# daooshee/ReReVST-Code

Measured on AMD Instinct MI355X. Metric: stylized frames/sec at 512x512, 1 style, higher is better.
Workload: dtype f32

## Files before the change

### rerevst-code_amd/csrc/conv_f43.h

```cpp
#pragma once
#include "conv_wino.h"

#ifndef F43_ABL
#define F43_ABL 0
#endif
#ifndef F43_SPAN
#define F43_SPAN 28
#endif

typedef float f32x2 __attribute__((ext_vector_type(2)));

struct F43Geo {
    static constexpr int NT = 256;
    static constexpr int NPOS = 36;
    static constexpr int RAW_ROW_BYTES = 4 * 9 * 32;
    static constexpr int RAW_PIECES = 34 * 4 * 9 * 2;
    static constexpr int RAW_IT = (RAW_PIECES + NT - 1) / NT;
    static constexpr int RAW_BYTES = RAW_IT * NT * 16;
    static constexpr int U_BYTES = NPOS * 32 * 8 * 4;
    static constexpr int U_IT = U_BYTES / 16 / NT;
    static constexpr int SMEM = 2 * RAW_BYTES + 2 * U_BYTES + WINO_PAR_BYTES;
};

__device__ __forceinline__ f32x2 p2sub(const f32x2 a, const f32x2 b) {
    f32x2 r;
    asm("v_pk_add_f32 %0, %1, %2 neg_lo:[0,1] neg_hi:[0,1]" : "=v"(r) : "v"(a), "v"(b));
    return r;
}
template <int IMM>
__device__ __forceinline__ f32x2 lds_rd64(unsigned addr) {
    static_assert(IMM >= 0 && IMM < 65536, "ds_read offset is a 16-bit unsigned immediate");
    f32x2 r;
    asm volatile("ds_read_b64 %0, %1 offset:%2" : "=v"(r) : "v"(addr), "i"(IMM));
    return r;
}

template <bool AG>
__device__ __forceinline__ void mfma_acc(f32x4& acc, const float a, const float b) {
    if constexpr (AG) asm volatile("v_mfma_f32_16x16x4_f32 %0, %1, %2, %0" : "+a"(acc) : "v"(a), "v"(b));
    else asm volatile("v_mfma_f32_16x16x4_f32 %0, %1, %2, %0" : "+v"(acc) : "v"(a), "v"(b));
}
template <bool AG>
__device__ __forceinline__ void mfma_zero(f32x4& acc, const float a, const float b) {
    if constexpr (AG) asm volatile("v_mfma_f32_16x16x4_f32 %0, %1, %2, 0" : "=a"(acc) : "v"(a), "v"(b));
    else asm volatile("v_mfma_f32_16x16x4_f32 %0, %1, %2, 0" : "=v"(acc) : "v"(a), "v"(b));
}

constexpr float F43_A = 0.75f, F43_B = 1.5f;
constexpr float F43_A2 = F43_A * F43_A, F43_B2 = F43_B * F43_B, F43_P = F43_A2 * F43_B2, F43_S = F43_A2 + F43_B2;
constexpr float F43_A3 = F43_A2 * F43_A, F43_B3 = F43_B2 * F43_B;
constexpr unsigned f43_bits(float f) { return __builtin_bit_cast(unsigned, f); }

struct F43Tmp { f32x2 a, b, c, f, g; };
struct F43K { unsigned long long b2, a2, p, s, a, b; };
__device__ __forceinline__ F43K f43_load_k() {
    F43K k;
    asm volatile("s_mov_b64 %0, %6\n\ts_mov_b64 %1, %7\n\ts_mov_b64 %2, %8\n\ts_mov_b64 %3, %9\n\ts_mov_b64 %4, %10\n\ts_mov_b64 %5, %11"
                 : "=s"(k.b2), "=s"(k.a2), "=s"(k.p), "=s"(k.s), "=s"(k.a), "=s"(k.b)
                 : "i"(f43_bits(F43_B2)), "i"(f43_bits(F43_A2)), "i"(f43_bits(F43_P)), "i"(f43_bits(F43_S)), "i"(f43_bits(F43_A)), "i"(f43_bits(F43_B)));
    return k;
}
template <bool NEG>
__device__ __forceinline__ void fmak3s(f32x2& r0, f32x2& r1, f32x2& r2, const f32x2 x0, const f32x2 x1, const f32x2 x2,
                                       const f32x2 c0, const f32x2 c1, const f32x2 c2, const unsigned long long ks) {
    if constexpr (NEG)
        asm volatile("v_pk_fma_f32 %0, %4, %3, %7 op_sel_hi:[1,0,1] neg_lo:[0,1,0] neg_hi:[0,1,0]\n\tv_pk_fma_f32 %1, %5, %3, %8 op_sel_hi:[1,0,1] neg_lo:[0,1,0] neg_hi:[0,1,0]\n\t"
                     "v_pk_fma_f32 %2, %6, %3, %9 op_sel_hi:[1,0,1] neg_lo:[0,1,0] neg_hi:[0,1,0]"
                     : "=&v"(r0), "=&v"(r1), "=&v"(r2) : "s"(ks), "v"(x0), "v"(x1), "v"(x2), "v"(c0), "v"(c1), "v"(c2));
    else
        asm volatile("v_pk_fma_f32 %0, %4, %3, %7 op_sel_hi:[1,0,1]\n\tv_pk_fma_f32 %1, %5, %3, %8 op_sel_hi:[1,0,1]\n\tv_pk_fma_f32 %2, %6, %3, %9 op_sel_hi:[1,0,1]"
                     : "=&v"(r0), "=&v"(r1), "=&v"(r2) : "s"(ks), "v"(x0), "v"(x1), "v"(x2), "v"(c0), "v"(c1), "v"(c2));
}
template <int LB, class LineFn>
__device__ __forceinline__ void f43_in3s(LineFn&& L, const F43K& k) {
    F43Tmp t[3];
    using N0 = std::integral_constant<int, LB>; using N1 = std::integral_constant<int, LB + 1>; using N2 = std::integral_constant<int, LB + 2>;
    using I0 = std::integral_constant<int, 0>; using I1 = std::integral_constant<int, 1>; using I2 = std::integral_constant<int, 2>;
    using I3 = std::integral_constant<int, 3>; using I4 = std::integral_constant<int, 4>; using I5 = std::integral_constant<int, 5>;
#define F43_D(J) L(N0{}, I##J{}), L(N1{}, I##J{}), L(N2{}, I##J{})
#define F43_T(M) t[0].M, t[1].M, t[2].M
    fmak3s<true>(F43_T(a), F43_D(2), F43_D(4), k.b2);
    fmak3s<true>(F43_T(b), F43_D(1), F43_D(3), k.b2);
    fmak3s<true>(F43_T(c), F43_D(2), F43_D(4), k.a2);
    fmak3s<true>(F43_T(f), F43_D(1), F43_D(3), k.a2);
    fmak3s<false>(F43_T(g), F43_D(0), F43_D(4), k.p);
    fmak3s<true>(F43_D(0), F43_D(2), F43_T(g), k.s);
    fmak3s<false>(F43_T(g), F43_D(1), F43_D(5), k.p);
    fmak3s<true>(F43_D(5), F43_D(3), F43_T(g), k.s);
    fmak3s<false>(F43_D(1), F43_T(b), F43_T(a), k.a);
    fmak3s<true>(F43_D(2), F43_T(b), F43_T(a), k.a);
    fmak3s<false>(F43_D(3), F43_T(f), F43_T(c), k.b);
    fmak3s<true>(F43_D(4), F43_T(f), F43_T(c), k.b);
#undef F43_D
#undef F43_T
}
__device__ __forceinline__ void f43_out(const f32x2 m0, const f32x2 m1, const f32x2 m2, const f32x2 m3, const f32x2 m4, const f32x2 m5,
                                        f32x2& y0, f32x2& y1, f32x2& y2, f32x2& y3) {
    f32x2 s1, d1, s2, d2;
    unsigned long long ks;
    asm volatile(
        "v_pk_add_f32 %[s1], %[m1], %[m2]\n\t"
        "v_pk_add_f32 %[d1], %[m1], %[m2] neg_lo:[0,1] neg_hi:[0,1]\n\t"
        "v_pk_add_f32 %[s2], %[m3], %[m4]\n\t"
        "v_pk_add_f32 %[d2], %[m3], %[m4] neg_lo:[0,1] neg_hi:[0,1]\n\t"
        "v_pk_add_f32 %[y0], %[m0], %[s1]\n\t"
        "s_mov_b64 %[k], %[ka]\n\t"
        "v_pk_mul_f32 %[y1], %[d1], %[k] op_sel_hi:[1,0]\n\t"
        "s_mov_b64 %[k], %[ka2]\n\t"
        "v_pk_mul_f32 %[y2], %[s1], %[k] op_sel_hi:[1,0]\n\t"
        "s_mov_b64 %[k], %[ka3]\n\t"
        "v_pk_fma_f32 %[y3], %[d1], %[k], %[m5] op_sel_hi:[1,0,1]\n\t"
        "v_pk_add_f32 %[y0], %[y0], %[s2]\n\t"
        "s_mov_b64 %[k], %[kb]\n\t"
        "v_pk_fma_f32 %[y1], %[d2], %[k], %[y1] op_sel_hi:[1,0,1]\n\t"
        "s_mov_b64 %[k], %[kb2]\n\t"
        "v_pk_fma_f32 %[y2], %[s2], %[k], %[y2] op_sel_hi:[1,0,1]\n\t"
        "s_mov_b64 %[k], %[kb3]\n\t"
        "v_pk_fma_f32 %[y3], %[d2], %[k], %[y3] op_sel_hi:[1,0,1]"
        : [y0] "=&v"(y0), [y1] "=&v"(y1), [y2] "=&v"(y2), [y3] "=&v"(y3), [s1] "=&v"(s1), [d1] "=&v"(d1), [s2] "=&v"(s2), [d2] "=&v"(d2), [k] "=&s"(ks)
        : [m0] "v"(m0), [m1] "v"(m1), [m2] "v"(m2), [m3] "v"(m3), [m4] "v"(m4), [m5] "v"(m5),
          [ka] "i"(f43_bits(F43_A)), [ka2] "i"(f43_bits(F43_A2)), [ka3] "i"(f43_bits(F43_A3)),
          [kb] "i"(f43_bits(F43_B)), [kb2] "i"(f43_bits(F43_B2)), [kb3] "i"(f43_bits(F43_B3)));
}

#ifndef P8_PAD
#define P8_PAD 6
#define P8_COL0 4
#endif
template <int EPI, int LAY = 0>
__global__ __launch_bounds__(256, 1) void conv_f43_k(const ConvP) {
    static_assert(!(EPI & E_RES), "same-resolution residuals are not needed by the layers this kernel serves");
    constexpr bool INP8 = (LAY & 1) != 0, OUTP8 = (LAY & 2) != 0;
    const ConvPK p0 = conv_args();
    auto wp_of = [](const ConvPK k) { return k->Wi + 2 + (INP8 ? P8_PAD : 0); };
    const int WP = wp_of(p0);
    using G = F43Geo;
    constexpr int ABL = F43_ABL;
    constexpr int RAW_BYTES = G::RAW_BYTES, U_BYTES = G::U_BYTES, NT = G::NT, NPOS = G::NPOS;
    extern __shared__ __attribute__((aligned(16))) char smem[];
    const int tid = threadIdx.x;
    const int wave = __builtin_amdgcn_readfirstlane(tid >> 6);
    const int lane = tid & 63, t = lane & 15, q = lane >> 4;
    const int tr = t >> 3, tc = t & 7;
    const int nchunks = p0->Cin >> 3;

    struct Item { int tx, ty, b, nt; };
    Item cur, nxt, dlt;
    {
        const ConvPK p = p0;
        const int n_ntiles = p->Cout >> 5;
        const int GD = gridDim.x, w = blockIdx.x;
        int pix, dpix;
        if (p->xcd_slabs) {
            const int PT = (GD >> 3) / n_ntiles;
            pix = (w & 7) * PT + (w >> 3) / n_ntiles; dpix = 8 * PT;
            cur.nt = (w >> 3) % n_ntiles; dlt.nt = 0;
        } else {
            cur.nt = w % n_ntiles; pix = w / n_ntiles;
            dlt.nt = GD % n_ntiles; dpix = GD / n_ntiles;
        }
        cur.tx = pix % p->tiles_x; cur.ty = (pix / p->tiles_x) % p->tiles_y; cur.b = pix / (p->tiles_x * p->tiles_y);
        dlt.tx = dpix % p->tiles_x; dlt.ty = (dpix / p->tiles_x) % p->tiles_y; dlt.b = dpix / (p->tiles_x * p->tiles_y);
    }
    auto advance = [&](const ConvPK p, const Item& a) {
        const int n_ntiles = p->Cout >> 5;
        Item r = a;
        r.nt += dlt.nt;
        int carry = 0;
        if (r.nt >= n_ntiles) { r.nt -= n_ntiles; carry = 1; }
        r.tx += dlt.tx + carry;
        if (r.tx >= p->tiles_x) { r.tx -= p->tiles_x; r.ty += 1; }
        r.ty += dlt.ty;
        if (r.ty >= p->tiles_y) { r.ty -= p->tiles_y; r.b += 1; }
        r.b += dlt.b;
        return r;
    };
    auto in_of = [&](const ConvPK p, const Item& a) {
        const int WP = wp_of(p);
        const size_t img_floats = (size_t)(p->Hi + 2) * WP * p->Cin;
        return p->in + (size_t)a.b * img_floats + (size_t)(((a.ty + p->ty0) * 32) * WP + (a.tx + p->tx0) * 32 + (INP8 ? P8_COL0 - 1 : 0)) * (INP8 ? 8 : p->Cin);
    };
    const size_t plane_floats = (size_t)(p0->Hi + 2) * WP * 8;
    auto lim_of = [&](const ConvPK p, const Item& a) {
        const int WP = wp_of(p);
        const long rows_left = (long)(p->Hi + 2) - (long)(a.ty + p->ty0) * 32;
        const long n = (rows_left * WP - (long)(a.tx + p->tx0) * 32 - (INP8 ? P8_COL0 - 1 : 0)) * (INP8 ? 8 : p->Cin) * 4;
        return (int)(n > 0x7fffffffL ? 0x7fffffffL : n);
    };
    auto w_of = [&](const ConvPK p, const Item& a) { return p->wpk + (size_t)a.nt * nchunks * (U_BYTES / 4); };
    int asrc[G::RAW_IT];
#pragma unroll
    for (int it = 0; it < G::RAW_IT; ++it) {
        int e = it * NT + tid;
        if (e >= G::RAW_PIECES) e = 0;
        const int half = e & 1, xd = (e >> 1) % 9, ph = ((e >> 1) / 9) & 3, y = (e >> 1) / 36;
        const int x = 4 * xd + ph, par = (y >> 2) & 1;
        asrc[it] = ((y * WP + x) * (INP8 ? 8 : p0->Cin) + 4 * (half ^ par)) * 4;
        if (ABL & 64) asrc[it] = (it * NT + tid) * 16;
    }
    bool have = cur.b < p0->B, have_nxt = false;
    const float* in_t = in_of(p0, cur);
    const float* w_t = w_of(p0, cur);
    int lim_t = lim_of(p0, cur);
    const float* in_n = in_t;
    const float* w_n = w_t;
    int lim_n = lim_t;
    auto stage_u = [&](int chunk) {
        char* udst = smem + 2 * RAW_BYTES + (chunk & 1) * U_BYTES;
#pragma unroll
        for (int it = 0; it < G::U_IT; ++it) bufld16(w_t, udst + (it * NT + wave * 64) * 16, tid * 16, chunk * U_BYTES + it * NT * 16);
    };
    auto stage_raw = [&](int chunk) {
        char* rdst = smem + (chunk & 1) * RAW_BYTES;
        const rsrc_t rs = make_rsrc(INP8 ? in_t + chunk * plane_floats : in_t, lim_t);
#pragma unroll
        for (int it = 0; it < G::RAW_IT; ++it) bufld16_rs(rs, rdst + (it * NT + wave * 64) * 16, asrc[it], INP8 ? 0 : chunk * 32);
    };
    char* const par = smem + 2 * RAW_BYTES + 2 * U_BYTES;
    auto stage_params = [&](int ntile, int img) {
        if (wave < 2) {
            const ConvPK p = conv_args();
            const int e = tid;
            const int row = e >> 3, col = (e & 7) * 4;
            const float* src = p->bias;
            int off = ntile * 32 + col;
            const int pb = img * p->par_bstride;
            if (row >= 1 && row <= 4) { src = (EPI & E_NORM1) ? p->n1 : p->bias; off += (EPI & E_NORM1) ? (row - 1) * p->Cout + pb : 0; }
            if (row >= 5 && row <= 8) { src = (EPI & E_NORM2) ? p->n2 : p->bias; off += (EPI & E_NORM2) ? (row - 5) * p->Cout + pb : 0; }
            if (row >= 9) { src = (EPI & E_NORM2) ? p->sty : p->bias; off += (EPI & E_NORM2) ? (row - 9) * p->Cout + pb : 0; }
            if (row > 10) { src = p->bias; off = ntile * 32; }
            glds16(src + off, par + wave * 1024);
        }
    };

    const unsigned lds0 = (unsigned)(size_t)(__attribute__((address_space(3))) char*)smem;
    const int y0 = 8 * wave + 4 * tr;
    const unsigned rawA = lds0 + y0 * G::RAW_ROW_BYTES + tc * 32 + ((q ^ (2 * (tr & 1))) << 3);
    const unsigned rawB = lds0 + y0 * G::RAW_ROW_BYTES + tc * 32 + ((q ^ (2 * ((tr & 1) ^ 1))) << 3);
    const unsigned offU = lds0 + 2 * RAW_BYTES + t * 64 + ((q ^ ((0 - (t >> 2)) & 3)) << 4);

#ifndef F43_NAG
#define F43_NAG 28
#endif
    constexpr int NAG = F43_NAG;
    f32x4 accA[NAG][2], accV[NPOS - NAG][2];
    int par_ntile = -1, par_img = -1;
    long long tl[10] = {0, 0, 0, 0, 0, 0, 0, 0, 0, 0}, tl_t = 0, pair_t = 0;
    const long long run_ck = (ABL & 16) ? clock64() : 0, run_rt = (ABL & 16) ? wall_clock64() : 0;
    auto tick = [&](int k) { if (ABL & 16) { const long long n = clock64(); tl[k] += n - tl_t; tl_t = n; } };
    f32x2 v[NPOS];
    f32x4 ur[2][6];
    auto full_transform = [&](f32x2 (&d)[NPOS]) {
        const F43K k = f43_load_k();
        auto col = [&](auto nc, auto jc) -> f32x2& { return d[decltype(nc)::value * 6 + decltype(jc)::value]; };
        auto row = [&](auto nc, auto jc) -> f32x2& { return d[decltype(jc)::value * 6 + decltype(nc)::value]; };
        f43_in3s<0>(col, k);
        f43_in3s<3>(col, k);
        f43_in3s<0>(row, k);
        f43_in3s<3>(row, k);
    };
    auto read_patch_col = [&](auto rbc, auto dxc) {
        constexpr int RB = decltype(rbc)::value, dx = decltype(dxc)::value;
        static_for([&](auto dyc) {
            constexpr int dy = decltype(dyc)::value;
            constexpr int off = RB + dy * G::RAW_ROW_BYTES + (dx & 3) * 288 + (dx >> 2) * 32;
            v[dx * 6 + dy] = lds_rd64<off>(dy < 4 ? rawA : rawB);
        }, std::make_integer_sequence<int, 6>{});
    };
    auto read_u_batch = [&](unsigned ub, auto bc, auto slotc) {
        constexpr int b = decltype(bc)::value, sl = decltype(slotc)::value;
        static_for([&](auto rc) {
            constexpr int r = decltype(rc)::value;
            ur[sl][r] = lds_rd128<(r * 6 + b) * 1024>(ub);
        }, std::make_integer_sequence<int, 6>{});
    };

    auto chunk_body = [&](int c, auto par_c, auto first_c, auto tail_c) {
        constexpr int PAR = decltype(par_c)::value;
        constexpr bool FIRST = decltype(first_c)::value;
        constexpr int TAIL = decltype(tail_c)::value;
        constexpr bool last = TAIL == 2;
        constexpr bool own_u = TAIL < 2, own_r = TAIL < 1;
        const rsrc_t rs_u = make_rsrc(own_u ? w_t : w_n);
        const int rchunk = own_r ? c + 2 : TAIL - 1;
        const rsrc_t rs_r = make_rsrc(INP8 ? (own_r ? in_t : in_n) + rchunk * plane_floats : (own_r ? in_t : in_n), own_r ? lim_t : lim_n);
        const int usoff = own_u ? (c + 1) * U_BYTES : 0;
        const int rsoff = INP8 ? 0 : rchunk * 32;
        int wb = wave * 1024;
        asm volatile("" : "+s"(wb));
        lds_char* const wdst = (lds_char*)smem + wb;
        lds_char* const udst = wdst + 2 * RAW_BYTES + (1 - PAR) * U_BYTES;
        lds_char* const rdst = wdst + PAR * RAW_BYTES;
        const unsigned ub = offU + PAR * U_BYTES;
        const unsigned ubn = offU + (1 - PAR) * U_BYTES;
        using RBt = std::integral_constant<int, (1 - PAR) * RAW_BYTES>;
        static_for([&](auto bc) {
            constexpr int b = decltype(bc)::value;
            if constexpr (b <= 1) asm volatile("s_waitcnt lgkmcnt(0)" ::: "memory");
            else if (last) asm volatile("s_waitcnt lgkmcnt(0)" ::: "memory");
            else asm volatile("s_waitcnt lgkmcnt(6)" ::: "memory");
            if constexpr (b < 5) read_u_batch(ub, std::integral_constant<int, b + 1>{}, std::integral_constant<int, (b + 1) & 1>{});
            static_for([&](auto rc) {
                constexpr int r = decltype(rc)::value, pos = r * 6 + b;
                constexpr int step = b * 6 + r;
                auto dma_req = [&](auto nc) {
                    constexpr int n = decltype(nc)::value;
                    if constexpr (n < G::RAW_IT) bufld16_rs(rs_r, rdst + n * NT * 16, asrc[n], rsoff);
                    else if constexpr (n < G::RAW_IT + G::U_IT) bufld16_rs(rs_u, udst + (n - G::RAW_IT) * NT * 16, tid * 16, usoff + (n - G::RAW_IT) * NT * 16);
                };
                {
                    constexpr int SPAN = F43_SPAN, NREQ = G::RAW_IT + G::U_IT;
                    constexpr int n = (step * NREQ + SPAN - 1) / SPAN;
                    if constexpr (n < NREQ && (n * SPAN) / NREQ == step) { if (!(ABL & 1)) dma_req(std::integral_constant<int, n>{}); }
                }
                if constexpr (r == 3) {
                    if constexpr (b >= 1) { if (!last) read_patch_col(RBt{}, std::integral_constant<int, b - 1>{}); }
                }
                constexpr bool AG = pos < NAG;
                f32x4 (&ac)[2] = *[&]() -> f32x4 (*)[2] { if constexpr (AG) return &accA[pos]; else return &accV[pos - NAG]; }();
                const f32x2 vv = v[b * 6 + r];
                const f32x4 uu = ur[b & 1][r];
                if constexpr (FIRST) { mfma_zero<AG>(ac[0], vv[0], uu[0]); mfma_zero<AG>(ac[1], vv[0], uu[2]); }
                else { mfma_acc<AG>(ac[0], vv[0], uu[0]); mfma_acc<AG>(ac[1], vv[0], uu[2]); }
                mfma_acc<AG>(ac[0], vv[1], uu[1]);
                mfma_acc<AG>(ac[1], vv[1], uu[3]);
            }, std::make_integer_sequence<int, 6>{});
        }, std::make_integer_sequence<int, 6>{});
        if (!last) read_patch_col(RBt{}, std::integral_constant<int, 5>{});
        tick(1);
        if (!(ABL & 2)) asm volatile("s_waitcnt vmcnt(0) lgkmcnt(0)\n\ts_barrier" ::: "memory");
        else asm volatile("s_waitcnt lgkmcnt(0)" ::: "memory");
        tick(3);
        if (!last) {
            read_u_batch(ubn, std::integral_constant<int, 0>{}, std::integral_constant<int, 0>{});
            if (!(ABL & 8)) full_transform(v);
        }
        tick(5);
    };

    auto next_patch = [&]() {
        static_for([&](auto dxc) { read_patch_col(std::integral_constant<int, 0>{}, dxc); }, std::make_integer_sequence<int, 6>{});
        read_u_batch(offU, std::integral_constant<int, 0>{}, std::integral_constant<int, 0>{});
        if (!(ABL & 2)) asm volatile("s_waitcnt lgkmcnt(0)\n\ts_barrier" ::: "memory");
        else asm volatile("s_waitcnt lgkmcnt(0)" ::: "memory");
        if (!(ABL & 8)) full_transform(v);
    };
    if (have) {
        stage_raw(0);
        stage_u(0);
        stage_raw(1);
        stage_params(cur.nt, cur.b);
        par_ntile = cur.nt; par_img = cur.b;
        __syncthreads();
        next_patch();
        __syncthreads();
    }
    if (ABL & 16) tl_t = clock64();
    while (have) {
        if (par_ntile != cur.nt || (conv_args()->par_bstride != 0 && par_img != cur.b)) {
            __syncthreads();
            stage_params(cur.nt, cur.b);
            par_ntile = cur.nt; par_img = cur.b;
        }
        tick(0);
        if (ABL & 16) pair_t = tl_t;
        using C0 = std::integral_constant<int, 0>; using C1 = std::integral_constant<int, 1>; using C2 = std::integral_constant<int, 2>;
        chunk_body(0, C0{}, std::true_type{}, C0{});
        chunk_body(1, C1{}, std::false_type{}, C0{});
        if (ABL & 16) { tl[6] += tl_t - pair_t; pair_t = tl_t; }
        for (int c = 2; c + 2 < nchunks; c += 2) {
            chunk_body(c, C0{}, std::false_type{}, C0{});
            chunk_body(c + 1, C1{}, std::false_type{}, C0{});
            if ((ABL & 16) && c == 2) tl[7] += tl_t - pair_t;
        }
        const int e_b = cur.b, e_ntile = cur.nt;
        int e_y0, e_x0;
        {
            const ConvPK pn = conv_args();
            e_y0 = (cur.ty + pn->ty0) * 32; e_x0 = (cur.tx + pn->tx0) * 32;
            nxt = advance(pn, cur);
            have_nxt = nxt.b < pn->B;
            in_n = have_nxt ? in_of(pn, nxt) : in_t;
            w_n = have_nxt ? w_of(pn, nxt) : w_t;
            lim_n = have_nxt ? lim_of(pn, nxt) : lim_t;
        }
        chunk_body(nchunks - 2, C0{}, std::false_type{}, C1{});
        chunk_body(nchunks - 1, C1{}, std::false_type{}, C2{});
        cur = nxt; have = have_nxt; in_t = in_n; w_t = w_n; lim_t = lim_n;
        asm volatile("s_nop 15\n\ts_nop 7");
        const ConvPK p = conv_args();
        int ln = lane;
        asm volatile("" : "+v"(ln));
        const int t = ln & 15, q = ln >> 4;
        auto ACC = [&](int i, int nb) -> f32x4 { return i < NAG ? accA[i][nb] : accV[i - NAG][nb]; };
        if (ABL & 32) {
            f32x4 s = ACC(0, 0);
#pragma unroll
            for (int i = 0; i < NPOS; ++i)
#pragma unroll
                for (int nb = 0; nb < 2; ++nb) if (i || nb) s += ACC(i, nb);
            if (s[0] + s[1] + s[2] + s[3] == 123.456f) p->out[tid] = s[0];
            if (have) next_patch();
            continue;
        }
        const int mr = q >> 1, mc0 = 4 * (q & 1);
        const int yb = e_y0 + 8 * wave + 4 * mr, xb0 = e_x0 + 4 * mc0;
        const unsigned lane_off = (unsigned)(((4 * (q >> 1)) * (p->W + 2) + 16 * (q & 1)) * p->Cout + 2 * t) * 4u;
        constexpr bool POOL = (EPI & E_POOL) != 0;
        const int Ho = POOL ? (p->H >> 1) : p->H, Wo = POOL ? (p->W >> 1) : p->W;
        constexpr int OP = OUTP8 ? P8_PAD : 0;
        char* const sb = OUTP8 ? (char*)(p->out + (size_t)e_b * (size_t)(Ho + 2) * (Wo + 2 + OP) * p->Cout + (size_t)e_ntile * 4 * (size_t)(Ho + 2) * (Wo + 2 + OP) * 8 +
                                         ((size_t)((POOL ? (e_y0 >> 1) + 4 * wave : e_y0 + 8 * wave) + 1) * (Wo + 2 + OP) + (POOL ? (e_x0 >> 1) : e_x0) + P8_COL0) * 8)
                               : (char*)(p->out + (size_t)e_b * (size_t)(Ho + 2) * (Wo + 2) * p->Cout +
                                 ((size_t)((POOL ? (e_y0 >> 1) + 4 * wave : e_y0 + 8 * wave) + 1) * (Wo + 2) + (POOL ? (e_x0 >> 1) : e_x0) + 1) * p->Cout + e_ntile * 32);
        int rowb = (Wo + 2) * p->Cout * 4, pixb = p->Cout * 4;
        unsigned st_off = POOL ? (unsigned)(((2 * mr) * (Wo + 2) + 2 * mc0) * p->Cout + 2 * t) * 4u : lane_off;
        if constexpr (OUTP8) {
            const unsigned plane = (unsigned)(Ho + 2) * (Wo + 2 + OP) * 32u;
            rowb = (Wo + 2 + OP) * 32; pixb = 32;
            st_off = (POOL ? (unsigned)((2 * mr) * (Wo + 2 + OP) + 2 * mc0) : (unsigned)((4 * (q >> 1)) * (p->W + 2 + OP) + 16 * (q & 1))) * 32u + (unsigned)(t >> 2) * plane + (unsigned)(t & 3) * 8u;
        }
        const bool interior = e_y0 + 32 <= p->H && e_x0 + 32 <= p->W;
        const char* const pl = par + 8 * t;
        const f32x2 bias = *(const f32x2*)(pl);
        f32x2 n1m, n1r, n1lo, n1hi, n2m, n2r, n2lo, n2hi, smean, sstd;
        if constexpr ((EPI & E_NORM1) != 0) { n1m = *(const f32x2*)(pl + 128); n1r = *(const f32x2*)(pl + 256); n1lo = *(const f32x2*)(pl + 384); n1hi = *(const f32x2*)(pl + 512); }
        if constexpr ((EPI & E_NORM2) != 0) {
            n2m = *(const f32x2*)(pl + 640); n2r = *(const f32x2*)(pl + 768); n2lo = *(const f32x2*)(pl + 896); n2hi = *(const f32x2*)(pl + 1024);
            smean = *(const f32x2*)(pl + 1152); sstd = *(const f32x2*)(pl + 1280);
        }
        f32x2 rres[4][2][2];
        if constexpr ((EPI & E_RES_UPS) != 0) {
            const float* const res_b = p->res + (size_t)e_b * (size_t)(p->Hr + 2) * (p->Wr + 2) * p->Cout + e_ntile * 32 + 2 * t;
#pragma unroll
            for (int e = 0; e < 4; ++e)
#pragma unroll
                for (int a = 0; a < 2; ++a)
#pragma unroll
                    for (int b2 = 0; b2 < 2; ++b2) {
                        const bool in = (yb + 2 * a < p->H) && (xb0 + 4 * e + 2 * b2 < p->W);
                        const int pix = in ? (((yb >> 1) + a + 1) * (p->Wr + 2) + ((xb0 + 4 * e) >> 1) + b2 + 1) : 0;
                        rres[e][a][b2] = *(const f32x2*)(res_b + (size_t)pix * p->Cout);
                    }
        }
        float lrk = 0.2f;
        asm volatile("" : "+s"(lrk));
        const f32x2 lrk2 = {lrk, lrk};
#pragma unroll
        for (int e = 0; e < 4; ++e) {
            auto PR = [&](int i) -> f32x2 { return f32x2{ACC(i, 0)[e], ACC(i, 1)[e]}; };
            f32x2 T[6][4];
#pragma unroll
            for (int r = 0; r < 6; ++r) {
                f43_out(PR(r * 6 + 0), PR(r * 6 + 1), PR(r * 6 + 2), PR(r * 6 + 3), PR(r * 6 + 4), PR(r * 6 + 5), T[r][0], T[r][1], T[r][2], T[r][3]);
                __builtin_amdgcn_sched_barrier(0);
            }
            f32x2 pool_prev[2];
#pragma unroll
            for (int j = 0; j < 4; ++j) {
                f32x2 o[4];
                f43_out(T[0][j], T[1][j], T[2][j], T[3][j], T[4][j], T[5][j], o[0], o[1], o[2], o[3]);
#pragma unroll
                for (int i = 0; i < 4; ++i) o[i] = o[i] + bias;
                if (EPI & E_RELU) {
#pragma unroll
                    for (int i = 0; i < 4; ++i) o[i] = f32x2{fmaxf(o[i][0], 0.f), fmaxf(o[i][1], 0.f)};
                }
                if (EPI & E_LRELU) {
#pragma unroll
                    for (int i = 0; i < 4; ++i) { const f32x2 s2 = o[i] * lrk2; o[i] = f32x2{fmaxf(o[i][0], s2[0]), fmaxf(o[i][1], s2[1])}; }
                }
                auto norm_clamp = [&](const f32x2 m, const f32x2 r, const f32x2 lo, const f32x2 hi) {
#pragma unroll
                    for (int i = 0; i < 4; ++i) o[i] = p2sub(o[i], m) * r;
#pragma unroll
                    for (int i = 0; i < 4; ++i) o[i] = f32x2{med3(o[i][0], lo[0], hi[0]), med3(o[i][1], lo[1], hi[1])};
                };
                if constexpr ((EPI & E_NORM1) != 0) norm_clamp(n1m, n1r, n1lo, n1hi);
                if constexpr ((EPI & E_RES_UPS) != 0) {
#pragma unroll
                    for (int i = 0; i < 4; ++i) o[i] = o[i] + rres[e][i >> 1][j >> 1];
                }
                if constexpr ((EPI & E_NORM2) != 0) {
                    norm_clamp(n2m, n2r, n2lo, n2hi);
#pragma unroll
                    for (int i = 0; i < 4; ++i) o[i] = __builtin_elementwise_fma(o[i], sstd, smean);
                }
                if constexpr (POOL) {
                    f32x2 m2[2];
#pragma unroll
                    for (int a = 0; a < 2; ++a) m2[a] = f32x2{fmaxf(o[2 * a][0], o[2 * a + 1][0]), fmaxf(o[2 * a][1], o[2 * a + 1][1])};
                    if ((j & 1) == 0) { pool_prev[0] = m2[0]; pool_prev[1] = m2[1]; continue; }
#pragma unroll
                    for (int a = 0; a < 2; ++a) m2[a] = f32x2{fmaxf(m2[a][0], pool_prev[a][0]), fmaxf(m2[a][1], pool_prev[a][1])};
                    char* const dst = sb + (2 * e + (j >> 1)) * pixb + st_off;
                    if (ABL & 4) { if (m2[0][0] == 123.456f) *(float*)dst = m2[0][0] + m2[1][0]; }
                    else if (interior) {
                        *(f32x2*)(dst) = m2[0]; *(f32x2*)(dst + rowb) = m2[1];
                    } else {
#pragma unroll
                        for (int a = 0; a < 2; ++a)
                            if ((yb >> 1) + a < Ho && ((xb0 + 4 * e) >> 1) + (j >> 1) < Wo) *(f32x2*)(dst + a * rowb) = m2[a];
                    }
                } else {
                    char* const dst = sb + (4 * e + j) * pixb + st_off;
                    if (ABL & 4) { if (o[0][0] == 123.456f) *(float*)dst = o[0][0] + o[1][0] + o[2][0] + o[3][0]; }
                    else if (interior) {
#pragma unroll
                        for (int i = 0; i < 4; ++i) *(f32x2*)(dst + i * rowb) = o[i];
                    } else {
#pragma unroll
                        for (int i = 0; i < 4; ++i)
                            if (yb + i < p->H && xb0 + 4 * e + j < p->W) *(f32x2*)(dst + i * rowb) = o[i];
                    }
                }
            }
        }
        tick(4);
        if (have) next_patch();
        tick(5);
    }
    if ((ABL & 16) && lane == 0) {
        tl[8] = clock64() - run_ck; tl[9] = wall_clock64() - run_rt;
#pragma unroll
        for (int k = 0; k < 10; ++k) conv_args()->dbg[(blockIdx.x * 4 + wave) * 10 + k] = tl[k];
    }
}

__global__ void pack_f43_k(const float* __restrict__ w, float* __restrict__ dst, int Cout, int Cin) {
    const size_t total = (size_t)Cout * Cin * 36;
    for (size_t i = blockIdx.x * (size_t)blockDim.x + threadIdx.x; i < total; i += (size_t)gridDim.x * blockDim.x) {
        size_t r = i;
        const int fl = (int)(r & 3); r >>= 2;
        const int slot = (int)(r & 3); r >>= 2;
        const int row = (int)(r & 15); r >>= 4;
        const int pos = (int)(r % 36); r /= 36;
        const int nchunks = Cin / 8;
        const int chunk = (int)(r % nchunks); r /= nchunks;
        const int n_tile = (int)r;
        const int pair = slot ^ ((0 - (row >> 2)) & 3);
        const int co = n_tile * 32 + 2 * row + (fl >> 1), ci = chunk * 8 + 2 * pair + (fl & 1);
        const float* g = w + ((size_t)co * Cin + ci) * 9;
        const int pr = pos / 6, pc = pos % 6;
        auto G3 = [](int rw, double g0, double g1, double g2) -> double {
            const double A = (double)F43_A, B = (double)F43_B;
            const double pt[5] = {0.0, A, -A, B, -B};
            if (rw == 5) return g2;
            double N = 1.0;
            for (int l = 0; l < 5; ++l) if (l != rw) N *= pt[rw] - pt[l];
            return (g0 + pt[rw] * g1 + pt[rw] * pt[rw] * g2) / N;
        };
        double rowv[3];
#pragma unroll
        for (int kx = 0; kx < 3; ++kx) rowv[kx] = G3(pr, g[0 * 3 + kx], g[1 * 3 + kx], g[2 * 3 + kx]);
        dst[i] = (float)G3(pc, rowv[0], rowv[1], rowv[2]);
    }
}
```

Baseline: 846.7.

## Prefetch residual tiles during last chunk and split epilogue into interior/edge paths

```diff
diff --git a/rerevst-code_amd/csrc/conv_f43.h b/rerevst-code_amd/csrc/conv_f43.h
--- a/rerevst-code_amd/csrc/conv_f43.h
+++ b/rerevst-code_amd/csrc/conv_f43.h
@@ -33,6 +33,20 @@
     f32x2 r;
     asm volatile("ds_read_b64 %0, %1 offset:%2" : "=v"(r) : "v"(addr), "i"(IMM));
     return r;
+}
+
+typedef unsigned u32x2 __attribute__((ext_vector_type(2)));
+__device__ __forceinline__ void bufst8(rsrc_t rs, const f32x2 v, unsigned voff, int soff) {
+#if defined(__HIP_DEVICE_COMPILE__)
+    __builtin_amdgcn_raw_buffer_store_b64(__builtin_bit_cast(u32x2, v), rs, (int)voff, soff, 0);
+#endif
+}
+__device__ __forceinline__ f32x2 bufld8(rsrc_t rs, unsigned voff, int soff) {
+#if defined(__HIP_DEVICE_COMPILE__)
+    return __builtin_bit_cast(f32x2, __builtin_amdgcn_raw_buffer_load_b64(rs, (int)voff, soff, 0));
+#else
+    return f32x2{};
+#endif
 }
 
 template <bool AG>
@@ -275,7 +289,7 @@
         }, std::make_integer_sequence<int, 6>{});
     };
 
-    auto chunk_body = [&](int c, auto par_c, auto first_c, auto tail_c) {
+    auto chunk_body = [&](int c, auto par_c, auto first_c, auto tail_c, auto&& mini_gap) {
         constexpr int PAR = decltype(par_c)::value;
         constexpr bool FIRST = decltype(first_c)::value;
         constexpr int TAIL = decltype(tail_c)::value;
@@ -315,6 +329,7 @@
                 }
                 if constexpr (r == 3) {
                     if constexpr (b >= 1) { if (!last) read_patch_col(RBt{}, std::integral_constant<int, b - 1>{}); }
+                    mini_gap(bc);
                 }
                 constexpr bool AG = pos < NAG;
                 f32x4 (&ac)[2] = *[&]() -> f32x4 (*)[2] { if constexpr (AG) return &accA[pos]; else return &accV[pos - NAG]; }();
@@ -365,12 +380,13 @@
         tick(0);
         if (ABL & 16) pair_t = tl_t;
         using C0 = std::integral_constant<int, 0>; using C1 = std::integral_constant<int, 1>; using C2 = std::integral_constant<int, 2>;
-        chunk_body(0, C0{}, std::true_type{}, C0{});
-        chunk_body(1, C1{}, std::false_type{}, C0{});
+        auto no_gap = [](auto) {};
+        chunk_body(0, C0{}, std::true_type{}, C0{}, no_gap);
+        chunk_body(1, C1{}, std::false_type{}, C0{}, no_gap);
         if (ABL & 16) { tl[6] += tl_t - pair_t; pair_t = tl_t; }
         for (int c = 2; c + 2 < nchunks; c += 2) {
-            chunk_body(c, C0{}, std::false_type{}, C0{});
-            chunk_body(c + 1, C1{}, std::false_type{}, C0{});
+            chunk_body(c, C0{}, std::false_type{}, C0{}, no_gap);
+            chunk_body(c + 1, C1{}, std::false_type{}, C0{}, no_gap);
             if ((ABL & 16) && c == 2) tl[7] += tl_t - pair_t;
         }
         const int e_b = cur.b, e_ntile = cur.nt;
@@ -384,10 +400,32 @@
             w_n = have_nxt ? w_of(pn, nxt) : w_t;
             lim_n = have_nxt ? lim_of(pn, nxt) : lim_t;
         }
-        chunk_body(nchunks - 2, C0{}, std::false_type{}, C1{});
-        chunk_body(nchunks - 1, C1{}, std::false_type{}, C2{});
+        chunk_body(nchunks - 2, C0{}, std::false_type{}, C1{}, no_gap);
+        f32x2 rres_h[4][2][2];
+        if constexpr ((EPI & E_RES_UPS) != 0) {
+            const ConvPK pr = conv_args();
+            const bool fetch = e_y0 + 32 <= pr->H && e_x0 + 32 <= pr->W && !(ABL & 128);
+            int lr = lane;
+            asm volatile("" : "+v"(lr));
+            const int WR = pr->Wr + 2;
+            const float* const res_u = pr->res + (size_t)e_b * (size_t)(pr->Hr + 2) * WR * pr->Cout + e_ntile * 32 +
+                                       ((size_t)((e_y0 >> 1) + 4 * wave + 1) * WR + (e_x0 >> 1) + 1) * pr->Cout;
+            const rsrc_t rs_r = make_rsrc(res_u, fetch ? 0x7fffffff : 0);
+            const unsigned r_off = (unsigned)((2 * (lr >> 5) * WR + 8 * ((lr >> 4) & 1)) * pr->Cout + 2 * (lr & 15)) * 4u;
+            const int rstep = pr->Cout * 4, rrow = WR * rstep;
+            chunk_body(nchunks - 1, C1{}, std::false_type{}, C2{}, [&](auto bc) {
+                constexpr int e = decltype(bc)::value - 1;
+                if constexpr (e >= 0 && e < 4) {
+#pragma unroll
+                    for (int a = 0; a < 2; ++a)
+#pragma unroll
+                        for (int b2 = 0; b2 < 2; ++b2) rres_h[e][a][b2] = bufld8(rs_r, r_off, a * rrow + (2 * e + b2) * rstep);
+                }
+            });
+        } else chunk_body(nchunks - 1, C1{}, std::false_type{}, C2{}, no_gap);
         cur = nxt; have = have_nxt; in_t = in_n; w_t = w_n; lim_t = lim_n;
         asm volatile("s_nop 15\n\ts_nop 7");
+        __builtin_amdgcn_sched_barrier(0);
         const ConvPK p = conv_args();
         int ln = lane;
         asm volatile("" : "+v"(ln));
@@ -429,26 +467,51 @@
             n2m = *(const f32x2*)(pl + 640); n2r = *(const f32x2*)(pl + 768); n2lo = *(const f32x2*)(pl + 896); n2hi = *(const f32x2*)(pl + 1024);
             smean = *(const f32x2*)(pl + 1152); sstd = *(const f32x2*)(pl + 1280);
         }
-        f32x2 rres[4][2][2];
-        if constexpr ((EPI & E_RES_UPS) != 0) {
-            const float* const res_b = p->res + (size_t)e_b * (size_t)(p->Hr + 2) * (p->Wr + 2) * p->Cout + e_ntile * 32 + 2 * t;
-#pragma unroll
-            for (int e = 0; e < 4; ++e)
-#pragma unroll
-                for (int a = 0; a < 2; ++a)
-#pragma unroll
-                    for (int b2 = 0; b2 < 2; ++b2) {
-                        const bool in = (yb + 2 * a < p->H) && (xb0 + 4 * e + 2 * b2 < p->W);
-                        const int pix = in ? (((yb >> 1) + a + 1) * (p->Wr + 2) + ((xb0 + 4 * e) >> 1) + b2 + 1) : 0;
-                        rres[e][a][b2] = *(const f32x2*)(res_b + (size_t)pix * p->Cout);
-                    }
-        }
         float lrk = 0.2f;
         asm volatile("" : "+s"(lrk));
         const f32x2 lrk2 = {lrk, lrk};
+        auto epilogue = [&](auto interior_c) {
+        constexpr bool INTERIOR = decltype(interior_c)::value;
+        unsigned so = st_off;
+        if constexpr (INTERIOR) asm volatile("; conv_f43_k epilogue: interior form" : "+v"(so));
+        else asm volatile("; conv_f43_k epilogue: edge form" : "+v"(so));
+        const rsrc_t rs_o = make_rsrc(sb);
+        const int rowb2 = 2 * rowb, rowb3 = 3 * rowb;
+        f32x2 rres[4][2][2];
+        if constexpr ((EPI & E_RES_UPS) != 0) {
+            if constexpr (INTERIOR) {
+#pragma unroll
+                for (int e = 0; e < 4; ++e)
+#pragma unroll
+                    for (int a = 0; a < 2; ++a)
+#pragma unroll
+                        for (int b2 = 0; b2 < 2; ++b2) {
+                            rres[e][a][b2] = rres_h[e][a][b2];
+                            if (ABL & 128) rres[e][a][b2] = f32x2{0.25f, -0.25f};
+                        }
+            } else {
+                const float* const res_b = p->res + (size_t)e_b * (size_t)(p->Hr + 2) * (p->Wr + 2) * p->Cout + e_ntile * 32 + 2 * t;
+#pragma unroll
+                for (int e = 0; e < 4; ++e)
+#pragma unroll
+                    for (int a = 0; a < 2; ++a)
+#pragma unroll
+                        for (int b2 = 0; b2 < 2; ++b2) {
+                            const bool in = (yb + 2 * a < p->H) && (xb0 + 4 * e + 2 * b2 < p->W);
+                            const int pix = in ? (((yb >> 1) + a + 1) * (p->Wr + 2) + ((xb0 + 4 * e) >> 1) + b2 + 1) : 0;
+                            rres[e][a][b2] = *(const f32x2*)(res_b + (size_t)pix * p->Cout);
+                        }
+            }
+        }
 #pragma unroll
         for (int e = 0; e < 4; ++e) {
-            auto PR = [&](int i) -> f32x2 { return f32x2{ACC(i, 0)[e], ACC(i, 1)[e]}; };
+            auto RD = [&](int i, int nb) -> float {
+                if (i >= NAG) return accV[i - NAG][nb][e];
+                float x;
+                asm volatile("v_accvgpr_read_b32 %0, %1" : "=v"(x) : "a"(accA[i][nb][e]));
+                return x;
+            };
+            auto PR = [&](int i) -> f32x2 { return f32x2{RD(i, 0), RD(i, 1)}; };
             f32x2 T[6][4];
 #pragma unroll
             for (int r = 0; r < 6; ++r) {
@@ -493,22 +556,26 @@
                     if ((j & 1) == 0) { pool_prev[0] = m2[0]; pool_prev[1] = m2[1]; continue; }
 #pragma unroll
                     for (int a = 0; a < 2; ++a) m2[a] = f32x2{fmaxf(m2[a][0], pool_prev[a][0]), fmaxf(m2[a][1], pool_prev[a][1])};
-                    char* const dst = sb + (2 * e + (j >> 1)) * pixb + st_off;
-                    if (ABL & 4) { if (m2[0][0] == 123.456f) *(float*)dst = m2[0][0] + m2[1][0]; }
-                    else if (interior) {
-                        *(f32x2*)(dst) = m2[0]; *(f32x2*)(dst + rowb) = m2[1];
+                    const int k = 2 * e + (j >> 1);
+                    if (ABL & 4) { if (m2[0][0] == 123.456f) *(float*)(sb + k * pixb + so) = m2[0][0] + m2[1][0]; }
+                    else if constexpr (INTERIOR) {
+                        bufst8(rs_o, m2[0], OUTP8 ? so + k * 32 : so, OUTP8 ? 0 : k * pixb);
+                        bufst8(rs_o, m2[1], OUTP8 ? so + k * 32 : so, OUTP8 ? rowb : k * pixb + rowb);
                     } else {
+                        char* const dst = sb + k * pixb + so;
 #pragma unroll
                         for (int a = 0; a < 2; ++a)
                             if ((yb >> 1) + a < Ho && ((xb0 + 4 * e) >> 1) + (j >> 1) < Wo) *(f32x2*)(dst + a * rowb) = m2[a];
                     }
                 } else {
-                    char* const dst = sb + (4 * e + j) * pixb + st_off;
-                    if (ABL & 4) { if (o[0][0] == 123.456f) *(float*)dst = o[0][0] + o[1][0] + o[2][0] + o[3][0]; }
-                    else if (interior) {
-#pragma unroll
-                        for (int i = 0; i < 4; ++i) *(f32x2*)(dst + i * rowb) = o[i];
+                    const int k = 4 * e + j;
+                    if (ABL & 4) { if (o[0][0] == 123.456f) *(float*)(sb + k * pixb + so) = o[0][0] + o[1][0] + o[2][0] + o[3][0]; }
+                    else if constexpr (INTERIOR) {
+                        const int rows[4] = {0, rowb, rowb2, rowb3};
+#pragma unroll
+                        for (int i = 0; i < 4; ++i) bufst8(rs_o, o[i], OUTP8 ? so + k * 32 : so, OUTP8 ? rows[i] : k * pixb + rows[i]);
                     } else {
+                        char* const dst = sb + k * pixb + so;
 #pragma unroll
                         for (int i = 0; i < 4; ++i)
                             if (yb + i < p->H && xb0 + 4 * e + j < p->W) *(f32x2*)(dst + i * rowb) = o[i];
@@ -516,6 +583,12 @@
                 }
             }
         }
+        };
+        int He = p->H;
+        asm volatile("" : "+s"(He));
+        const bool edge = e_y0 + 32 > He || e_x0 + 32 > p->W;
+        if (interior) epilogue(std::true_type{});
+        if (edge) epilogue(std::false_type{});
         tick(4);
         if (have) next_patch();
         tick(5);
```

Result: slower. 836.0 (-1.3%).
